# mgtools/DCTdomain

Measured on AMD Instinct MI355X. Metric: DCT fingerprints/sec on L=500 D=1280, higher is better.
Workload: dtype f64

## Files before the change

### dctdomain_amd/csrc/dctfp.hip

```cpp
#include "dctfp.h"

#include <hip/hip_runtime.h>

#include <dlfcn.h>
#include <execinfo.h>
#include <signal.h>
#include <unistd.h>

#include <algorithm>
#include <cmath>
#include <cstdarg>
#include <cstdio>
#include <cstring>
#include <map>
#include <mutex>
#include <new>
#include <string>
#include <unordered_map>
#include <vector>

#include "launch.h"
#include "reccut_kernel.hip.h"

using namespace dctfp;
// ... 2007 lines not shown
                    sp.row_end = row;
                    sp.stripe = stripe++;
                }
            }
        }
    }
    const int64_t used_stripes = s_fill;
    rc = tables.upload(up_bytes, stream, all_bytes);
    if (rc) return rc;
    const TopkJob* djobs = (const TopkJob*)tables.dev();
    const bool long_beside = n_long > 0 && used_stripes > 0 && n_short > 0;
    hipStream_t long_stream = stream;
    if (long_beside) {
        rc = ctx->ensure_cut_streams();
        if (rc == DCTFP_OK) rc = fork.fork(ctx->cut_fork);
        if (rc == DCTFP_OK) rc = fork.branch(ctx->cut[0], &long_stream);
        if (rc) return rc;
    }
    if (n_short > 0) {
        if (ctx->opt_topk_kernel != 1) {
            if (ctx->opt_topk_kernel == 0) {
                constexpr int kSmallK = 1400;
                bool any_small = false, any_large = false;
                for (int32_t q = 0; q < n_short; ++q) (h[q].k <= kSmallK ? any_small : any_large) = true;
                if (any_small)
                    hipLaunchKernelGGL((contact_topk1_kernel<8>), dim3((unsigned)n_short), dim3(512), 0, stream, djobs, out_i, out_j, out_v, out_n, 0, kSmallK);
                if (any_large)
                    hipLaunchKernelGGL((contact_topk1_kernel<16>), dim3((unsigned)n_short), dim3(1024), 0, stream, djobs, out_i, out_j, out_v, out_n,
                                       kSmallK + 1, 0x7fffffff);
            }
            hipLaunchKernelGGL(contact_topk2_kernel, dim3((unsigned)n_short), dim3(1024), 0, stream, djobs, out_i, out_j, out_v, out_n,
                               ctx->opt_topk_kernel == 0 ? 1 : 0);
            hipLaunchKernelGGL(contact_topk_kernel, dim3((unsigned)n_short), dim3(1024), 0, stream, djobs, out_i, out_j, out_v, out_n, 1);
        } else {
            hipLaunchKernelGGL(contact_topk_kernel, dim3((unsigned)n_short), dim3(1024), 0, stream, djobs, out_i, out_j, out_v, out_n, 0);
        }
        HIP_TRY(hipGetLastError());
    }
    if (n_long > 0 && used_stripes > 0) {
        stream = long_stream;
        const TopkJob* dlong = djobs + n_short;
        const TopkStripe* dstripes = (const TopkStripe*)(tables.dev() + off_stripe);
        const int32_t* dfirst = (const int32_t*)(tables.dev() + off_first);
        TopkState* dstate = (TopkState*)(tables.dev() + off_state);
        int32_t* dties = (int32_t*)(tables.dev() + off_ties);
        for (int shift = 24; shift >= 0; shift -= 8) {
            hipLaunchKernelGGL(topk_hist_kernel, dim3((unsigned)used_stripes), dim3(1024), 0, stream, dlong, dstripes, dstate, shift);
            hipLaunchKernelGGL(topk_pick_kernel, dim3((unsigned)n_long), dim3(64), 0, stream, dlong, dstate, shift, out_n);
        }
        hipLaunchKernelGGL(topk_collect_kernel, dim3((unsigned)used_stripes), dim3(1024), 0, stream, dlong, dstripes, dstate, dties, out_i,
                           out_j, out_v);
        hipLaunchKernelGGL(topk_ties_kernel, dim3((unsigned)used_stripes), dim3(64), 0, stream, dlong, dstripes, dstate, dties, dfirst,
                           out_i, out_j, out_v);
        HIP_TRY(hipGetLastError());
    }
    rc = fork.join();
    return rc ? rc : tables.release();
} DCTFP_GUARD("dctfp_contact_topk")

int dctfp_contact_sort(dctfp_ctx* ctx, const void* const* maps, const int64_t* ld, const int32_t* n_res, int32_t n_prot,
                       double t, int32_t* out_i, int32_t* out_j, float* out_v, const int64_t* out_offs, uint8_t* sorted,
                       void* stream_v) try {
    if (!ctx || !maps || !ld || !n_res || !out_i || !out_j || !out_v || !out_offs || !sorted)
        return fail(DCTFP_ERR_INVALID, "dctfp_contact_sort: NULL argument");
    std::lock_guard<std::mutex> lock(ctx->mu);
    if (n_prot < 0) return fail(DCTFP_ERR_INVALID, "dctfp_contact_sort: negative count");
    if (n_prot == 0) return DCTFP_OK;
    hipStream_t stream = (hipStream_t)stream_v;
    HIP_TRY(hipSetDevice(ctx->device));
    static const int kNet[4] = {2048, 4096, 8192, 16384};
    std::vector<int32_t> group[4];
    for (int32_t p = 0; p < n_prot; ++p) {
        const int64_t k = dctfp_contact_count(n_res[p], t);
        sorted[p] = 1;
        if (k <= 1) continue;
        if (n_res[p] > 65536 || k > kNet[3]) {
            sorted[p] = 0;
            continue;
        }
        if (!maps[p] || ld[p] < n_res[p]) return fail(DCTFP_ERR_INVALID, "dctfp_contact_sort: protein %d: bad map", p);
        int g = 0;
        while (k > kNet[g]) ++g;
        group[g].push_back(p);
    }
    const size_t n_jobs = group[0].size() + group[1].size() + group[2].size() + group[3].size();
    if (n_jobs == 0) return DCTFP_OK;
    TableLease tables(ctx->ring, stream);
    int rc = tables.stage(n_jobs * sizeof(TopkJob));
    if (rc) return rc;
    TopkJob* h = (TopkJob*)tables.host();
    size_t q = 0;
    for (int g = 0; g < 4; ++g)
        for (int32_t p : group[g]) {
            h[q].map = (const float*)maps[p];
            h[q].ld = ld[p];
            h[q].n_res = n_res[p];
            h[q].k = (int32_t)dctfp_contact_count(n_res[p], t);
            h[q].out_off = out_offs[p];
            h[q].orig = p;
            h[q].reserved = 0;
            ++q;
        }
    rc = tables.upload(n_jobs * sizeof(TopkJob), stream);
    if (rc) return rc;
    const TopkJob* d = (const TopkJob*)tables.dev();
    size_t first = 0;
    for (int g = 0; g < 4; ++g) {
        const unsigned n = (unsigned)group[g].size();
        if (n == 0) continue;
        if (g == 0) hipLaunchKernelGGL((contact_sort_kernel<2048>), dim3(n), dim3(1024), 0, stream, d + first, out_i, out_j, out_v);
        else if (g == 1) hipLaunchKernelGGL((contact_sort_kernel<4096>), dim3(n), dim3(1024), 0, stream, d + first, out_i, out_j, out_v);
        else if (g == 2) hipLaunchKernelGGL((contact_sort_kernel<8192>), dim3(n), dim3(1024), 0, stream, d + first, out_i, out_j, out_v);
        else hipLaunchKernelGGL((contact_sort_kernel<16384>), dim3(n), dim3(1024), 0, stream, d + first, out_i, out_j, out_v);
        HIP_TRY(hipGetLastError());
        first += n;
    }
    return tables.release();
} DCTFP_GUARD("dctfp_contact_sort")

int64_t dctfp_reccut_room(int32_t n_res) {
    const int64_t doms = n_res > 0 ? n_res / kCutMinSize + 1 : 1;
    return 2 + doms + 2 * (2 * doms + 1);
}

int dctfp_reccut(dctfp_ctx* ctx, const int32_t* n_res, int32_t n_prot, const int32_t* ci, const int32_t* cj, const float* cv,
                 const int64_t* offs, double cut1, double cut2, int32_t* out, const int64_t* out_offs, void* stream_v) try {
    if (!ctx || !n_res || !offs || !out || !out_offs) return fail(DCTFP_ERR_INVALID, "dctfp_reccut: NULL argument");
    std::lock_guard<std::mutex> lock(ctx->mu);
    if (n_prot < 0) return fail(DCTFP_ERR_INVALID, "dctfp_reccut: negative count");
    if (n_prot == 0) return DCTFP_OK;
    hipStream_t stream = (hipStream_t)stream_v;
    HIP_TRY(hipSetDevice(ctx->device));
    std::vector<int32_t> order((size_t)n_prot);
    int32_t count[kCutClasses] = {};
    std::vector<uint8_t> cls((size_t)n_prot);
    size_t adj_total = 0;
    for (int32_t p = 0; p < n_prot; ++p) {
        const int64_t nc = offs[p + 1] - offs[p];
        if (n_res[p] < 0 || nc < 0 || nc > 0x7fffffff || (nc > 0 && (!ci || !cj || !cv)))
            return fail(DCTFP_ERR_INVALID, "dctfp_reccut: protein %d: bad sizes", p);
        if (out_offs[p + 1] - out_offs[p] < 4) return fail(DCTFP_ERR_INVALID, "dctfp_reccut: protein %d: output room below 4", p);
        cls[(size_t)p] = (uint8_t)reccut_class_of(n_res[p], nc);
        ++count[cls[(size_t)p]];
        adj_total += 2 * (size_t)nc + 6 * (size_t)std::max(n_res[p], 0);
    }
    int32_t first[kCutClasses];
    {
        int32_t at[kCutClasses], run = 0;
        for (int c = 0; c < kCutClasses; ++c) {
            first[c] = at[c] = run;
            run += count[c];
        }
        for (int32_t p = 0; p < n_prot; ++p) order[(size_t)at[cls[(size_t)p]]++] = p;
    }
    const size_t stack_ints = (size_t)kCutStack * kCutNodeInts;
    const size_t ws_bytes = align_up(adj_total * sizeof(uint32_t), 16) + (size_t)n_prot * stack_ints * sizeof(int32_t);
    Hold cut_ws{ctx->cut_ws, stream};
    int rc = cut_ws.take(ws_bytes, stream);
    if (rc) return rc;
    TableLease tables(ctx->ring, stream);
    Fork fork(stream);
    rc = tables.stage((size_t)n_prot * sizeof(CutJob));
    if (rc) return rc;
    CutJob* h = (CutJob*)tables.host();
    uint32_t* adj = (uint32_t*)cut_ws.p();
    int32_t* stacks = (int32_t*)((char*)cut_ws.p() + align_up(adj_total * sizeof(uint32_t), 16));
    size_t adj_at = 0;
    for (int32_t q = 0; q < n_prot; ++q) {
        const int32_t p = order[(size_t)q];
        const int64_t nc = offs[p + 1] - offs[p];
        CutJob& j = h[q];
        j.ci = ci ? ci + offs[p] : nullptr;
        j.cj = cj ? cj + offs[p] : nullptr;
        j.cv = cv ? cv + offs[p] : nullptr;
        j.adj = adj + adj_at;
        adj_at += 2 * (size_t)nc + 6 * (size_t)std::max(n_res[p], 0);
        j.stack = stacks + (size_t)q * stack_ints;
        j.out = out + out_offs[p];
        j.timing = nullptr;
#ifdef DCTFP_CUT_TIMING
        j.timing = ctx->degenerate + 1;
#endif
        j.n_contacts = (int32_t)nc;
        j.n_res = n_res[p];
        j.out_cap = (int32_t)std::min<int64_t>(out_offs[p + 1] - out_offs[p], 0x7fffffff);
        j.reserved = 0;
    }
    rc = tables.upload((size_t)n_prot * sizeof(CutJob), stream);
    if (rc) return rc;
    const CutJob* d = (const CutJob*)tables.dev();
    int n_used = 0;
    for (int c = 0; c < kCutClasses; ++c) n_used += count[c] > 0 ? 1 : 0;
    const bool beside = n_used > 1;
    if (beside) {
        rc = ctx->ensure_cut_streams();
        if (rc == DCTFP_OK) rc = fork.fork(ctx->cut_fork);
        if (rc) return rc;
    }
    for (int c = 0; c < kCutClasses; ++c) {
        if (count[c] == 0) continue;
        hipStream_t s = stream;
        if (beside && c > 0) rc = fork.branch(ctx->cut[c - 1], &s);
        if (rc) return rc;
        for (int32_t done = 0; done < count[c]; done += 65535 * 16) {
            const unsigned n = (unsigned)std::min<int32_t>(count[c] - done, 65535 * 16);
            LaunchError le;
            rc = launcher_rc(launch_reccut(c, d + first[c] + done, n, cut1, cut2, s, &le), le);
            if (rc) return rc;
            HIP_TRY(hipGetLastError());
        }
        rc = fork.join();
        if (rc) return rc;
    }
    rc = cut_ws.give_back();
    return rc ? rc : tables.release();
} DCTFP_GUARD("dctfp_reccut")

}

namespace {
struct StitchOnce {
    const float* prev;
    int64_t ld_prev;
    int32_t n_skip;
};
int stitch_impl(dctfp_ctx* ctx, const dctfp_stitch_job* jobs, int64_t n_jobs, int32_t n_cols, int32_t square, void* stream_v,
                const StitchOnce* once = nullptr) {
    if (n_jobs < 0 || (!square && n_cols < 1)) return fail(DCTFP_ERR_INVALID, "dctfp_stitch: bad count");
    if (n_jobs == 0) return DCTFP_OK;
    if (n_jobs > 65535 * 64) return fail(DCTFP_ERR_LIMIT, "dctfp_stitch: too many windows in one call");
    hipStream_t stream = (hipStream_t)stream_v;
    HIP_TRY(hipSetDevice(ctx->device));
    int32_t max_level = 0;
    bool vec4 = !square && n_cols % 4 == 0;
    for (int64_t i = 0; i < n_jobs; ++i) {
        const dctfp_stitch_job& j = jobs[i];
        if (!aligned16(j.src) || !aligned16(j.dst) || (j.ld_src % 4) || (j.ld_dst % 4)) vec4 = false;
        if (once && once[i].prev && (!aligned16(once[i].prev) || (once[i].ld_prev % 4))) vec4 = false;
        if (!j.src || !j.dst || j.n_rows < 1 || j.n_avg < 0 || j.n_avg > j.n_rows || j.level < 0 ||
            j.ld_src < (square ? j.n_rows : n_cols) || j.ld_dst < (square ? j.n_rows : n_cols))
            return fail(DCTFP_ERR_INVALID, "dctfp_stitch: window %lld is malformed", (long long)i);
        if (j.level == 0 && j.n_avg != 0) return fail(DCTFP_ERR_INVALID, "dctfp_stitch: window %lld: level 0 cannot average", (long long)i);
        max_level = std::max(max_level, j.level);
    }
    if (once) max_level = 0;
    TableLease tables(ctx->ring, stream);
    int rc = tables.stage((size_t)n_jobs * sizeof(StitchJob));
    if (rc) return rc;
    StitchJob* h = (StitchJob*)tables.host();
    std::vector<int64_t> start((size_t)max_level + 2, 0);
    for (int64_t i = 0; i < n_jobs; ++i) start[(size_t)(once ? 0 : jobs[i].level) + 1] += 1;
    for (int32_t l = 0; l <= max_level; ++l) start[(size_t)l + 1] += start[(size_t)l];
    std::vector<int64_t> fill(start.begin(), start.end() - 1);
    std::vector<int32_t> max_rows((size_t)max_level + 1, 0);
    for (int64_t i = 0; i < n_jobs; ++i) {
        const dctfp_stitch_job& j = jobs[i];
        const int32_t level = once ? 0 : j.level;
        StitchJob& o = h[fill[(size_t)level]++];
        o.src = (const float*)j.src;
        o.dst = (float*)j.dst;
        o.n_rows = j.n_rows;
        o.n_avg = j.n_avg;
        o.ld_src = j.ld_src;
        o.ld_dst = j.ld_dst;
        o.prev = once ? once[i].prev : nullptr;
        o.ld_prev = once ? once[i].ld_prev : 0;
        o.n_skip = once ? once[i].n_skip : 0;
        o.reserved = 0;
        max_rows[(size_t)level] = std::max(max_rows[(size_t)level], j.n_rows);
    }
    rc = tables.upload((size_t)n_jobs * sizeof(StitchJob), stream);
    if (rc) return rc;
    const StitchJob* d = (const StitchJob*)tables.dev();
    for (int32_t l = 0; l <= max_level; ++l) {
        int64_t cnt = start[(size_t)l + 1] - start[(size_t)l];
        int64_t done = 0;
        while (done < cnt) {
            const unsigned ny = (unsigned)std::min<int64_t>(cnt - done, 65535);
            dim3 grid((unsigned)((max_rows[(size_t)l] + 15) / 16), ny);
            if (square) hipLaunchKernelGGL(stitch_contacts_kernel, grid, dim3(256), 0, stream, d + start[(size_t)l] + done);
            else if (vec4) hipLaunchKernelGGL((stitch_rows_kernel<true>), grid, dim3(256), 0, stream, d + start[(size_t)l] + done, n_cols);
            else hipLaunchKernelGGL((stitch_rows_kernel<false>), grid, dim3(256), 0, stream, d + start[(size_t)l] + done, n_cols);
            HIP_TRY(hipGetLastError());
            done += ny;
        }
    }
    return tables.release();
}

}

extern "C" {

int dctfp_stitch(dctfp_ctx* ctx, const dctfp_stitch_job* jobs, int64_t n_jobs, int32_t n_cols, int32_t square,
                 void* stream_v) try {
    if (!ctx || (!jobs && n_jobs > 0)) return fail(DCTFP_ERR_INVALID, "dctfp_stitch: NULL argument");
    std::lock_guard<std::mutex> lock(ctx->mu);
    return stitch_impl(ctx, jobs, n_jobs, n_cols, square, stream_v);
} DCTFP_GUARD("dctfp_stitch")

int dctfp_stitch_sizes(const int32_t* win_rows, const int64_t* seq_win, int64_t n_seq, int32_t step, int32_t square,
                       int64_t* out_rows) try {
    if (!win_rows || !seq_win || !out_rows || n_seq < 0 || step < 0) return fail(DCTFP_ERR_INVALID, "dctfp_stitch_sizes: bad argument");
    for (int64_t s = 0; s < n_seq; ++s) {
        const int64_t n = seq_win[s + 1] - seq_win[s];
        out_rows[s] = stitch_geometry(win_rows + seq_win[s], n, step, square != 0, [](int64_t, int64_t, int32_t) {});
// ... 558 lines not shown
```

### dctdomain_amd/csrc/reccut_kernel.hip.h

```cpp
#pragma once

#include <hip/hip_runtime.h>
#include <stdint.h>

namespace dctfp {

constexpr int kCutMinTerminal = 10;
constexpr int kCutMinSize = 22;
constexpr int kCutMaxSeg = 24;
constexpr int kCutStack = 24;
constexpr int kCutNodeInts = 4 + 2 * kCutMaxSeg + kCutMaxSeg;

struct CutJob {
    const int32_t* ci;
    const int32_t* cj;
    const float* cv;
    uint32_t* adj;
    int32_t* stack;
    int32_t* out;
    unsigned long long* timing;
    int32_t n_contacts;
    int32_t n_res;
    int32_t out_cap;
    int32_t reserved;
};

__host__ __device__ inline int contact_weight_exact(float p) {
    const double n6 = rint((double)p * 1.0e6);
    const double v = n6 / 1.0e6;
#ifdef __HIP_DEVICE_COMPILE__
    return (int)__dadd_rn(__dmul_rn(v, 100.0), 0.5);
#else
    volatile double prod = v * 100.0;
    return (int)(prod + 0.5);
#endif
}

template <int kCutThreads>
__device__ inline void block_scan_inclusive(int32_t* __restrict__ v, int n, int32_t* __restrict__ wave_tot) {
    const int tid = threadIdx.x, lane = tid & 63, wave = tid >> 6;
    constexpr int NW = kCutThreads / 64;
    int base = 0;
    for (int c0 = 0; c0 < n; c0 += kCutThreads) {
        const int p = c0 + tid;
        int x = p < n ? v[p] : 0;
#pragma unroll
        for (int off = 1; off < 64; off <<= 1) {
            const int up = __shfl_up(x, off);
            x += lane >= off ? up : 0;
        }
        if (lane == 63) wave_tot[wave] = x;
        __syncthreads();
        int before = base;
        for (int w = 0; w < wave; ++w) before += wave_tot[w];
        int total = 0;
        for (int w = 0; w < NW; ++w) total += wave_tot[w];
        if (p < n) v[p] = x + before;
        base += total;
        __syncthreads();
    }
}

__device__ inline bool cut_better(double a, int i, int j, double b, int bi, int bj) {
    return a < b || (a == b && (i < bi || (i == bi && j < bj)));
}

template <int CAP, int ECAP, int kCutThreads, int RB, int KMAX>
__global__ __launch_bounds__(kCutThreads, 4 ) void reccut_kernel(const CutJob* __restrict__ jobs, double cut1, double cut2) {
    extern __shared__ int32_t lds[];
    int32_t* __restrict__ idx = lds;
    int32_t* __restrict__ tmp = idx + CAP;
    int32_t* __restrict__ pos = tmp + CAP;
    int32_t* __restrict__ off = pos + CAP;
    int32_t* __restrict__ foff = off + CAP + 1;
    int32_t* __restrict__ A = foff + CAP + 1;
    int32_t* __restrict__ B = A + CAP + 1;
    uint32_t* __restrict__ fwd = reinterpret_cast<uint32_t*>(B + CAP + 2);
    int32_t* __restrict__ node = reinterpret_cast<int32_t*>(fwd + ECAP);
    int32_t* __restrict__ kid = node + kCutNodeInts;
    int32_t* __restrict__ wtot = kid + 2 * kCutNodeInts;
    int32_t* __restrict__ U = wtot + 32;
    uint8_t* __restrict__ M = reinterpret_cast<uint8_t*>(U + RB * (CAP / 64 + 1));
    int32_t* __restrict__ INITX = reinterpret_cast<int32_t*>(M + RB * CAP);
    auto INIT = [&](int b) -> int32_t* { return b == 0 ? pos : INITX + (b - 1) * CAP; };
    int32_t* __restrict__ WT = INITX + (KMAX > 2 ? KMAX - 2 : 0) * CAP;
    constexpr int RBS = RB / KMAX;
    constexpr int SLOTS = (KMAX * (CAP / 64) / 2 + (CAP / 64) / 2 + 2 * KMAX + kCutThreads / 64 - 1) / (kCutThreads / 64);
    static_assert(RB % KMAX == 0 && RBS % 4 == 0 && RBS * KMAX * 1 <= kCutThreads, "tile rows: RBS rows of each of KMAX bands");
    int32_t* __restrict__ misc = wtot + 16;
    __shared__ double red_ave[kCutThreads / 64];
    __shared__ int red_i[kCutThreads / 64], red_j[kCutThreads / 64];

    const CutJob job = jobs[blockIdx.x];
    const int tid = threadIdx.x, lane = tid & 63, wave = tid >> 6;
    const int L = job.n_res;
    int32_t* __restrict__ out = job.out;
#ifdef DCTFP_CUT_TIMING
    unsigned long long tl_prev = __builtin_amdgcn_s_memrealtime(), tl_acc[11] = {0, 0, 0, 0, 0, 0, 0, 0, 0, 0, 0};
#define CUT_T(k)                                                          \
    do {                                                                  \
        const unsigned long long now_ = __builtin_amdgcn_s_memrealtime(); \
        tl_acc[k] += now_ - tl_prev;                                      \
        tl_prev = now_;                                                   \
    } while (0)
#define CUT_T_OUT()                                                                     \
    do {                                                                                \
        if (tid == 0 && job.timing)                                                     \
            for (int q_ = 0; q_ < 11; ++q_) atomicAdd(job.timing + q_, tl_acc[q_]);      \
    } while (0)
#else
#define CUT_T(k)
#define CUT_T_OUT()
#endif
    if (L < kCutMinSize) {
        if (tid == 0 && job.out_cap >= 4) {
            out[0] = 1;
            out[1] = 1;
            out[2] = 0;
            out[3] = L - 1;
        } else if (tid == 0 && job.out_cap >= 1) {
            out[0] = -1;
        }
        return;
    }
    if (L > CAP || (int64_t)job.n_contacts + 3ll * L > ECAP || job.out_cap < 4) {
        if (tid == 0 && job.out_cap >= 1) out[0] = -1;
        return;
    }
    if (tid < 16) misc[tid] = 0;
    for (int q = tid; q < RB * CAP / 4; q += kCutThreads) reinterpret_cast<uint32_t*>(M)[q] = 0;
    for (int q = tid; q < RB * (CAP / 64 + 1); q += kCutThreads) U[q] = 0;
    __syncthreads();

    for (int r = tid; r < L; r += kCutThreads) {
        int d = 0;
        for (int s = 1; s <= 3; ++s) d += (r - s >= 0 ? 1 : 0) + (r + s < L ? 1 : 0);
        tmp[r] = d;
        idx[r] = r;
        pos[r] = -1;
    }
    __syncthreads();
    for (int c = tid; c < job.n_contacts; c += kCutThreads) {
        const int i = job.ci[c], j = job.cj[c];
        const float p = job.cv[c];
        if (i < 0 || j < 0 || i >= L || j >= L || !(fabsf(p) < 1.0e6f)) {
            misc[4] = 1;
            continue;
        }
        const int d = i > j ? i - j : j - i;
        if (d == 0 || d <= 3) continue;
        if (contact_weight_exact(p) == 0) continue;
        atomicAdd(&tmp[i], 1);
        atomicAdd(&tmp[j], 1);
    }
    __syncthreads();
    for (int r = tid; r < L; r += kCutThreads) A[r] = tmp[r];
    __syncthreads();
    block_scan_inclusive<kCutThreads>(A, L, wtot);
    for (int r = tid; r < L; r += kCutThreads) {
        const int begin = A[r] - tmp[r];
        off[r] = begin;
        if (r == L - 1) off[L] = A[r];
        int at = begin;
        for (int s = 1; s <= 3; ++s) {
            if (r - s >= 0) job.adj[at++] = (uint32_t)(r - s) | (100u << 16);
            if (r + s < L) job.adj[at++] = (uint32_t)(r + s) | (100u << 16);
        }
        B[r] = at;
    }
    __syncthreads();
    if (misc[4] == 0)
        for (int c = tid; c < job.n_contacts; c += kCutThreads) {
            const int i = job.ci[c], j = job.cj[c];
            const int d = i > j ? i - j : j - i;
            if (d <= 3) continue;
            const int w = contact_weight_exact(job.cv[c]);
            if (w == 0) continue;
            if (w < 0 || w > 255) {
                misc[4] = 1;
                continue;
            }
            job.adj[atomicAdd(&B[i], 1)] = (uint32_t)j | ((uint32_t)w << 16);
            job.adj[atomicAdd(&B[j], 1)] = (uint32_t)i | ((uint32_t)w << 16);
        }
    __threadfence_block();
    __syncthreads();
    if (misc[4] != 0) {
        if (tid == 0) out[0] = -1;
        return;
    }
    CUT_T(0);
    if (tid == 0) {
        node[0] = 0;
        node[1] = L;
        node[2] = 1;
        node[3] = 0;
        node[4] = 0;
        node[5] = L - 1;
        misc[9] = 1;
        misc[10] = 0;
        misc[11] = 0;
    }
    __syncthreads();

    for (;;) {
        const int first = node[0], V = node[1];
        int32_t* __restrict__ ix = idx + first;
        for (int p = tid; p < V; p += kCutThreads) pos[ix[p]] = p;
        __syncthreads();
        for (int p = tid; p < V; p += kCutThreads) {
            const int r = ix[p];
            int pre = 0, post = 0, fd = 0;
            for (int e = off[r]; e < off[r + 1]; ++e) {
                const uint32_t a = job.adj[e];
                const int q = pos[a & 0xffffu];
                if (q >= 0) {
                    const int w = (int)(a >> 16);
                    if (q < p) pre += w;
                    else {
                        post += w;
                        ++fd;
                    }
                }
            }
            A[p] = pre;
            B[p] = post;
            foff[p] = fd;
            tmp[p] = fd;
        }
        __syncthreads();
        block_scan_inclusive<kCutThreads>(foff, V, wtot);
        const int n_fwd = foff[V - 1];
        if (n_fwd > ECAP) {
            if (tid == 0) out[0] = -1;
            return;
        }
        for (int p = tid; p < V; p += kCutThreads) {
            const int r = ix[p];
            int at = foff[p] - tmp[p];
            for (int e = off[r]; e < off[r + 1]; ++e) {
                const uint32_t a = job.adj[e];
                const int q = pos[a & 0xffffu];
                if (q > p) fwd[at++] = (uint32_t)q | (a & 0xffff0000u);
            }
        }
        __syncthreads();
        for (int p = tid; p < V; p += kCutThreads) foff[p] = foff[p] - tmp[p];
        CUT_T(1);
        const int post0 = B[0];
        __syncthreads();
        if (tid == 0) {
            A[0] = 0;
            B[0] = 0;
        }
        __syncthreads();
        block_scan_inclusive<kCutThreads>(A, V, wtot);
        block_scan_inclusive<kCutThreads>(B, V, wtot);
        const int sum = B[V - 1] + post0;
        double b1 = 2.0;
        int b1i = 0x7fffffff;
        for (int i = tid; i < V; i += kCutThreads) {
            const int n1 = A[i], spost = B[i];
            const int n2 = sum - spost;
            if (i >= 1 && i < V - 2) {
                const int cutv = post0 + spost - n1;
                const double ave = ((double)cutv) * sum / n1 / n2;
                if (ave < 2.0 && cut_better(ave, i, 0, b1, b1i, 0)) {
                    b1 = ave;
                    b1i = i;
                }
            }
        }
        __syncthreads();
        for (int i = tid; i < V; i += kCutThreads) B[i] = sum - B[i];
        if (tid == 0) B[V] = 0;
        __syncthreads();
        int tj_keep[(CAP + kCutThreads - 1) / kCutThreads], ci_keep[(CAP + kCutThreads - 1) / kCutThreads];
#pragma unroll
        for (int m = 0; m < (CAP + kCutThreads - 1) / kCutThreads; ++m) {
            const int i = m * kCutThreads + tid;
            tj_keep[m] = i < V ? A[i] - B[i + 1] : 0;
            ci_keep[m] = i >= 1 && i < V ? B[i] - A[i - 1] : 0;
        }
        __syncthreads();
#pragma unroll
        for (int m = 0; m < (CAP + kCutThreads - 1) / kCutThreads; ++m) {
            const int i = m * kCutThreads + tid;
            if (i < V) {
                A[i] = tj_keep[m];
                B[i] = ci_keep[m];
            }
        }
        {
#pragma unroll
            for (int o = 32; o >= 1; o >>= 1) {
                const double oa = __shfl_xor(b1, o);
                const int oi = __shfl_xor(b1i, o);
                if (cut_better(oa, oi, 0, b1, b1i, 0)) {
                    b1 = oa;
                    b1i = oi;
                }
            }
            if (lane == 0) {
                red_ave[wave] = b1;
                red_i[wave] = b1i;
            }
        }
        __syncthreads();
        double best1 = 2.0;
        int cuts = 0;
        {
            int bi = 0x7fffffff;
            for (int w = 0; w < kCutThreads / 64; ++w)
                if (cut_better(red_ave[w], red_i[w], 0, best1, bi, 0)) {
                    best1 = red_ave[w];
                    bi = red_i[w];
                }
            if (bi != 0x7fffffff) cuts = bi + 1;
        }
        __syncthreads();
        CUT_T(2);
        double b2 = 2.0;
        int b2i = 0x7fffffff, b2j = 0x7fffffff;
        const bool small = sum > 0 && sum < (1 << 23);
        const float sum_f = (float)sum;
        const int j_end = V - kCutMinTerminal;
        constexpr int NG = CAP / 64, NWV = kCutThreads / 64;
        const int hi_top = j_end - 2;
        const int n_scan_rows = hi_top - kCutMinTerminal + 1;
        int K = n_scan_rows / 16;
        K = K < 1 ? 1 : (K > KMAX ? KMAX : K);
        int band_rows = n_scan_rows > 0 ? (n_scan_rows + K - 1) / K : RBS;
        band_rows = (band_rows + RBS - 1) / RBS * RBS;
        const int n_iter = n_scan_rows > 0 ? band_rows / RBS : 0;
        const int NGa = (j_end + 63) >> 6;
        auto band_top = [&](int b) { return hi_top - b * band_rows; };
        auto band_low = [&](int b) { return max(kCutMinTerminal, hi_top - (b + 1) * band_rows + 1); };
        if (KMAX > 1 && K > 1) {
            for (int b = 0; b < K - 1; ++b)
                for (int q = tid; q < V; q += kCutThreads) INIT(b)[q] = 0;
            __syncthreads();
            for (int a = tid; a <= hi_top; a += kCutThreads) {
                if (a < kCutMinTerminal + 1) continue;
                const int bb = (hi_top - a) / band_rows + 1;
                if (bb >= K) continue;
                const int e1 = foff[a] + tmp[a];
                for (int e = foff[a]; e < e1; ++e) {
                    const uint32_t ent = fwd[e];
                    atomicAdd(&INIT(bb - 1)[(int)(ent & 0xffffu)], (int)(ent >> 16));
                }
            }
            __syncthreads();
            {
                constexpr int PER = (CAP + kCutThreads - 1) / kCutThreads;
                int carry[KMAX > 1 ? KMAX - 1 : 1];
#pragma unroll
                for (int b = 0; b < KMAX - 1; ++b) carry[b] = 0;
#pragma unroll
                for (int m = 0; m < PER; ++m) {
                    const int q = m * kCutThreads + tid;
                    int x[KMAX > 1 ? KMAX - 1 : 1];
                    int run = 0;
#pragma unroll
                    for (int b = 0; b < KMAX - 1; ++b) {
                        run += (b < K - 1 && q < V) ? INIT(b)[q] : 0;
                        x[b] = run;
                    }
#pragma unroll
                    for (int off2 = 1; off2 < 64; off2 <<= 1) {
#pragma unroll
                        for (int b = 0; b < KMAX - 1; ++b) {
                            const int up = __shfl_up(x[b], off2);
                            x[b] += lane >= off2 ? up : 0;
                        }
                    }
                    if (lane == 63) {
#pragma unroll
                        for (int b = 0; b < KMAX - 1; ++b) WT[b * NWV + wave] = x[b];
                    }
                    __syncthreads();
#pragma unroll
                    for (int b = 0; b < KMAX - 1; ++b) {
                        int before = carry[b], total = 0;
                        for (int w = 0; w < NWV; ++w) {
                            const int t_w = WT[b * NWV + w];
                            before += w < wave ? t_w : 0;
                            total += t_w;
                        }
                        if (b < K - 1 && q < V) INIT(b)[q] = x[b] + before;
                        carry[b] += total;
                    }
                    __syncthreads();
                }
            }
        }
        int n_tasks = 0;
        int cum[KMAX + 1];
#pragma unroll
        for (int b = 0; b < KMAX; ++b) {
            cum[b] = n_tasks;
            if (b < K && n_scan_rows > 0 && band_top(b) >= kCutMinTerminal) {
                const int g_lo = (band_low(b) + 1) >> 6;
                n_tasks += max(0, NGa - g_lo);
            }
        }
        cum[KMAX] = n_tasks;
        int task_b[SLOTS], task_g[SLOTS], below[SLOTS];
#pragma unroll
        for (int sl = 0; sl < SLOTS; ++sl) {
            const int tau = wave + sl * NWV;
            int b = -1, g = 0;
            if (tau < n_tasks) {
#pragma unroll
                for (int bb = 0; bb < KMAX; ++bb)
                    if (tau >= cum[bb] && tau < cum[bb + 1]) {
                        b = bb;
                        g = ((band_low(bb) + 1) >> 6) + tau - cum[bb];
                    }
            }
            task_b[sl] = b;
            task_g[sl] = g;
            const int j = g * 64 + lane;
            below[sl] = (b >= 1 && j < j_end) ? INIT(b - 1)[j] : 0;
        }
        if (n_tasks > SLOTS * NWV) {
            if (tid == 0) out[0] = -1;
            return;
        }
        float best_f = 2.0f * 1.0001f;
        for (int it = 0; it < n_iter; ++it) {
            constexpr int FPR = kCutThreads / (KMAX * RBS) >= 8 ? 8 : kCutThreads / (KMAX * RBS);
            const int fill_t = tid / FPR, fill_b = fill_t / RBS;
            int fill_row = -1;
            if (fill_b < K) {
                const int r = band_top(fill_b) - it * RBS - (fill_t % RBS);
                if (r >= band_low(fill_b)) fill_row = r;
            }
            if (fill_row >= 0) {
                const int e1 = foff[fill_row] + tmp[fill_row];
                for (int e = foff[fill_row] + tid % FPR; e < e1; e += FPR) {
                    const uint32_t ent = fwd[e];
                    const int q = (int)(ent & 0xffffu);
                    M[fill_t * CAP + q] = (uint8_t)(ent >> 16);
                    atomicAdd(&U[fill_t * (NG + 1) + (q >> 6)], (int)(ent >> 16));
                }
            }
            __syncthreads();
            CUT_T(3);
#pragma unroll
            for (int sl = 0; sl < SLOTS; ++sl) {
                const int b = task_b[sl], g = task_g[sl];
                if (b < 0) continue;
                const int hi = band_top(b) - it * RBS;
                const int n_rows = min(RBS, hi - band_low(b) + 1);
                const int g0 = g * 64;
                if (n_rows <= 0 || g0 + 63 <= hi - n_rows + 1) continue;
                const int j = g0 + lane;
                const bool col_ok = j < j_end;
                const int tj = col_ok ? A[j] : 0;
                const int tr0 = b * RBS;
                int m_u = 0;
                if (lane < n_rows)
                    for (int k = 0; k < g; ++k) m_u += U[(tr0 + lane) * (NG + 1) + k];
                const int m_c = lane < n_rows ? B[hi - lane] : 0;
                int bl = below[sl];
                static_assert(RBS % 4 == 0, "rows go through four at a time");
                for (int t = 0; t < n_rows; t += 4) {
                    int x[4], ns2[4], cv[4], ns1[4];
                    bool maybe[4];
#pragma unroll
                    for (int k = 0; k < 4; ++k) x[k] = (int)M[(tr0 + t + k) * CAP + j];
#pragma unroll
                    for (int k = 0; k < 4; ++k) {
                        x[k] += __builtin_amdgcn_update_dpp(0, x[k], 0x111, 0xf, 0xf, true);
                        x[k] += __builtin_amdgcn_update_dpp(0, x[k], 0x112, 0xf, 0xf, true);
                        x[k] += __builtin_amdgcn_update_dpp(0, x[k], 0x114, 0xf, 0xf, true);
                        x[k] += __builtin_amdgcn_update_dpp(0, x[k], 0x118, 0xf, 0xf, true);
                        x[k] += __builtin_amdgcn_update_dpp(0, x[k], 0x142, 0xa, 0xf, false);
                        x[k] += __builtin_amdgcn_update_dpp(0, x[k], 0x143, 0xc, 0xf, false);
                    }
                    bool any = false;
#pragma unroll
                    for (int k = 0; k < 4; ++k) {
                        bl += x[k] + __builtin_amdgcn_readlane(m_u, min(t + k, 63));
                        const int i = hi - t - k;
                        ns2[k] = bl;
                        cv[k] = tj + __builtin_amdgcn_readlane(m_c, min(t + k, 63)) - 2 * bl;
                        ns1[k] = sum - cv[k] - bl;
                        maybe[k] = t + k < n_rows && col_ok && j - i >= kCutMinSize - 1 && ns1[k] > 0 && ns2[k] > 0;
                        if (small) maybe[k] = maybe[k] && (float)cv[k] * sum_f <= best_f * (float)ns1[k] * (float)ns2[k];
                        any |= maybe[k];
                    }
                    if (__builtin_amdgcn_ballot_w64(any) != 0) {
                        bool improved = false;
#pragma unroll
                        for (int k = 0; k < 4; ++k)
                            if (maybe[k]) {
                                const double ave = ((double)cv[k]) * sum / ns1[k] / ns2[k];
                                if (ave < 2.0 && cut_better(ave, hi - t - k, j, b2, b2i, b2j)) {
                                    b2 = ave;
                                    b2i = hi - t - k;
                                    b2j = j;
                                    improved = true;
                                }
                            }
                        if (__builtin_amdgcn_ballot_w64(improved) != 0) {
                            double wmin = b2;
#pragma unroll
                            for (int o = 32; o >= 1; o >>= 1) wmin = fmin(wmin, __shfl_xor(wmin, o));
                            best_f = (float)(wmin * 1.0001);
                        }
                    }
                }
                below[sl] = bl;
            }
            CUT_T(8);
            __syncthreads();
            CUT_T(9);
            if (fill_row >= 0) {
                const int e1 = foff[fill_row] + tmp[fill_row];
                for (int e = foff[fill_row] + tid % FPR; e < e1; e += FPR) {
                    const int q = (int)(fwd[e] & 0xffffu);
                    M[fill_t * CAP + q] = 0;
                    U[fill_t * (NG + 1) + (q >> 6)] = 0;
                }
            }
            __syncthreads();
            CUT_T(10);
        }
#pragma unroll
        for (int o = 32; o >= 1; o >>= 1) {
            const double oa = __shfl_xor(b2, o);
            const int oi = __shfl_xor(b2i, o), oj = __shfl_xor(b2j, o);
            if (cut_better(oa, oi, oj, b2, b2i, b2j)) {
                b2 = oa;
                b2i = oi;
                b2j = oj;
            }
        }
        if (lane == 0) {
            red_ave[wave] = b2;
            red_i[wave] = b2i;
            red_j[wave] = b2j;
        }
        __syncthreads();
        CUT_T(3);
        if (tid == 0) {
            double best2 = 2.0;
            int cuts1 = 0x7fffffff, cuts2 = 0x7fffffff;
            for (int w = 0; w < kCutThreads / 64; ++w)
                if (cut_better(red_ave[w], red_i[w], red_j[w], best2, cuts1, cuts2)) {
                    best2 = red_ave[w];
                    cuts1 = red_i[w];
                    cuts2 = red_j[w];
                }
            if (cuts1 == 0x7fffffff) cuts1 = cuts2 = 0;
            const int n_seg = node[2], n_site = node[3];
            const int32_t* __restrict__ segs = node + 4;
            const int32_t* __restrict__ sites = node + 4 + 2 * kCutMaxSeg;
            int action = 0;
            int32_t* __restrict__ k1 = kid;
            int32_t* __restrict__ k2 = kid + kCutNodeInts;
            int n1s = 0, n1c = 0, n2s = 0, n2c = 0;
            bool bad = false;
            auto seg_ok = [&](int c) { return c >= 0 && c < n_seg; };
            auto push_seg = [&](int32_t* __restrict__ k, int& n, int a, int b) {
                if (n >= kCutMaxSeg) {
                    bad = true;
                    return;
                }
                k[4 + 2 * n] = a;
                k[4 + 2 * n + 1] = b;
                ++n;
            };
            auto push_site = [&](int32_t* __restrict__ k, int& n, int v) {
                if (n >= kCutMaxSeg) {
                    bad = true;
                    return;
                }
                k[4 + 2 * kCutMaxSeg + n] = v;
                ++n;
            };
            if (best1 - cut1 <= best2 - cut2) {
                if (!(best1 > cut1 || cuts < kCutMinSize || V - cuts < kCutMinSize)) {
                    action = 1;
                    int c = 0;
                    while (c < n_site && sites[c] < cuts) {
                        if (!seg_ok(c)) bad = true;
                        else push_seg(k1, n1s, segs[2 * c], segs[2 * c + 1]);
                        push_site(k1, n1c, sites[c]);
                        ++c;
                        if (bad) break;
                    }
                    if (!bad && !seg_ok(c)) bad = true;
                    if (!bad) {
                        const int len1 = c == 0 ? cuts : cuts - sites[c - 1];
                        const int mf = segs[2 * c], ms = segs[2 * c + 1];
                        push_seg(k1, n1s, mf, mf + len1 - 1);
                        const int len2 = (n_site == 0 || c == n_site) ? V - cuts : sites[c] - cuts;
                        if (len2 > 0) {
                            push_seg(k2, n2s, ms - len2 + 1, ms);
                            if (c < n_site) push_site(k2, n2c, len2);
                        }
                        for (++c; c < n_seg; ++c) {
                            push_seg(k2, n2s, segs[2 * c], segs[2 * c + 1]);
                            if (c < n_site && len1 > 0) push_site(k2, n2c, len1);
                        }
                    }
                    k1[1] = cuts;
                    k2[1] = V - cuts;
                }
            } else {
                const int length = cuts2 - cuts1;
                if (!(best2 > cut2 || length < kCutMinSize || V - length < kCutMinSize)) {
                    action = 2;
                    const int ns = n_site;
                    const int tail = V - cuts2;
                    int c1 = -1, c2 = 0;
                    for (int i = ns - 1; i >= 0; --i) {
                        if (sites[i] < cuts2) c2 = i + 1;
                        if (sites[i] <= cuts1) {
                            c1 = i;
                            break;
                        }
                    }
                    auto cs_at = [&](int i) {
                        if (i == -1 && ns > 0) return 0;
                        if (i < 0 || i >= ns) {
                            bad = true;
                            return 0;
                        }
                        return sites[i];
                    };
                    const int len2 = c2 == 0 ? cuts2 : cuts2 - cs_at(c2 - 1);
                    if (!seg_ok(c2)) bad = true;
                    if (!bad) {
                        push_seg(k1, n1s, segs[2 * c2] + len2, segs[2 * c2 + 1]);
                        for (int i = c2 + 1; i <= ns && !bad; ++i) {
                            if (!seg_ok(i)) bad = true;
                            else push_seg(k1, n1s, segs[2 * i], segs[2 * i + 1]);
                        }
                        for (int i = c2; i < ns; ++i) push_site(k1, n1c, sites[i] - cuts2);
                        push_site(k1, n1c, tail);
                        for (int i = 0; i <= c1 && !bad; ++i) {
                            if (!seg_ok(i)) bad = true;
                            else push_seg(k1, n1s, segs[2 * i], segs[2 * i + 1]);
                            if (sites[i] != cuts1) push_site(k1, n1c, sites[i] + tail);
                        }
                    }
                    if (!bad) {
                        const int len1 = c1 >= 0 ? cuts1 - sites[c1] : cuts1;
                        ++c1;
                        if (len1 > 0) {
                            if (!seg_ok(c1)) bad = true;
                            else push_seg(k1, n1s, segs[2 * c1], segs[2 * c1] + len1 - 1);
                        }
                        if (!bad && c2 > c1) {
                            const int lhs = cs_at(c1 - 1) + len1, rhs = cs_at(c1);
                            if (!bad && lhs < rhs) {
                                if (!seg_ok(c1)) bad = true;
                                else push_seg(k2, n2s, segs[2 * c1] + len1, segs[2 * c1 + 1]);
                            }
                        }
                        for (int i = c1 + 1; i < c2 && !bad; ++i) {
                            if (!seg_ok(i)) bad = true;
                            else push_seg(k2, n2s, segs[2 * i], segs[2 * i + 1]);
                        }
                        if (!bad) {
                            if (c2 > c1 && len2 > 0) {
                                if (!seg_ok(c2)) bad = true;
                                else push_seg(k2, n2s, segs[2 * c2], segs[2 * c2] + len2 - 1);
                            } else if (c1 == c2) {
                                if (!seg_ok(c2)) bad = true;
                                else push_seg(k2, n2s, segs[2 * c2] + len1, segs[2 * c2] + len2 - 1);
                            }
                        }
                        for (int i = c1; i < c2 && !bad; ++i) {
                            const int v = cs_at(i) - cuts1;
                            if (!bad && v > 0) push_site(k2, n2c, v);
                        }
// ... 94 lines not shown
```

Before: 1.373 million.

## Pack row prefix scans, drop barriers, sort cut jobs by size

After: 1.373 million (median of 6 runs). No clear change (-0.0%).

```diff
diff --git a/dctdomain_amd/csrc/dctfp.hip b/dctdomain_amd/csrc/dctfp.hip
--- a/dctdomain_amd/csrc/dctfp.hip
+++ b/dctdomain_amd/csrc/dctfp.hip
@@ -2183,6 +2183,10 @@
             run += count[c];
         }
         for (int32_t p = 0; p < n_prot; ++p) order[(size_t)at[cls[(size_t)p]]++] = p;
+        for (int c = 0; c < kCutClasses; ++c)
+            std::stable_sort(order.begin() + first[c], order.begin() + first[c] + count[c], [&](int32_t a, int32_t b) {
+                return (int64_t)n_res[a] * n_res[a] > (int64_t)n_res[b] * n_res[b];
+            });
     }
     const size_t stack_ints = (size_t)kCutStack * kCutNodeInts;
     const size_t ws_bytes = align_up(adj_total * sizeof(uint32_t), 16) + (size_t)n_prot * stack_ints * sizeof(int32_t);
diff --git a/dctdomain_amd/csrc/reccut_kernel.hip.h b/dctdomain_amd/csrc/reccut_kernel.hip.h
--- a/dctdomain_amd/csrc/reccut_kernel.hip.h
+++ b/dctdomain_amd/csrc/reccut_kernel.hip.h
@@ -88,8 +88,8 @@
     constexpr int SLOTS = (KMAX * (CAP / 64) / 2 + (CAP / 64) / 2 + 2 * KMAX + kCutThreads / 64 - 1) / (kCutThreads / 64);
     static_assert(RB % KMAX == 0 && RBS % 4 == 0 && RBS * KMAX * 1 <= kCutThreads, "tile rows: RBS rows of each of KMAX bands");
     int32_t* __restrict__ misc = wtot + 16;
-    __shared__ double red_ave[kCutThreads / 64];
-    __shared__ int red_i[kCutThreads / 64], red_j[kCutThreads / 64];
+    __shared__ double red_ave[kCutThreads / 64], red1_ave[kCutThreads / 64];
+    __shared__ int red_i[kCutThreads / 64], red_j[kCutThreads / 64], red1_i[kCutThreads / 64];
 
     const CutJob job = jobs[blockIdx.x];
     const int tid = threadIdx.x, lane = tid & 63, wave = tid >> 6;
@@ -302,8 +302,8 @@
                 }
             }
             if (lane == 0) {
-                red_ave[wave] = b1;
-                red_i[wave] = b1i;
+                red1_ave[wave] = b1;
+                red1_i[wave] = b1i;
             }
         }
         __syncthreads();
@@ -312,13 +312,12 @@
         {
             int bi = 0x7fffffff;
             for (int w = 0; w < kCutThreads / 64; ++w)
-                if (cut_better(red_ave[w], red_i[w], 0, best1, bi, 0)) {
-                    best1 = red_ave[w];
-                    bi = red_i[w];
+                if (cut_better(red1_ave[w], red1_i[w], 0, best1, bi, 0)) {
+                    best1 = red1_ave[w];
+                    bi = red1_i[w];
                 }
             if (bi != 0x7fffffff) cuts = bi + 1;
         }
-        __syncthreads();
         CUT_T(2);
         double b2 = 2.0;
         int b2i = 0x7fffffff, b2j = 0x7fffffff;
@@ -430,6 +429,7 @@
         float best_f = 2.0f * 1.0001f;
         for (int it = 0; it < n_iter; ++it) {
             constexpr int FPR = kCutThreads / (KMAX * RBS) >= 8 ? 8 : kCutThreads / (KMAX * RBS);
+            static_assert(64 % FPR == 0, "a tile row's fill threads lie in one wave");
             const int fill_t = tid / FPR, fill_b = fill_t / RBS;
             int fill_row = -1;
             if (fill_b < K) {
@@ -468,16 +468,23 @@
                 for (int t = 0; t < n_rows; t += 4) {
                     int x[4], ns2[4], cv[4], ns1[4];
                     bool maybe[4];
-#pragma unroll
-                    for (int k = 0; k < 4; ++k) x[k] = (int)M[(tr0 + t + k) * CAP + j];
-#pragma unroll
-                    for (int k = 0; k < 4; ++k) {
-                        x[k] += __builtin_amdgcn_update_dpp(0, x[k], 0x111, 0xf, 0xf, true);
-                        x[k] += __builtin_amdgcn_update_dpp(0, x[k], 0x112, 0xf, 0xf, true);
-                        x[k] += __builtin_amdgcn_update_dpp(0, x[k], 0x114, 0xf, 0xf, true);
-                        x[k] += __builtin_amdgcn_update_dpp(0, x[k], 0x118, 0xf, 0xf, true);
-                        x[k] += __builtin_amdgcn_update_dpp(0, x[k], 0x142, 0xa, 0xf, false);
-                        x[k] += __builtin_amdgcn_update_dpp(0, x[k], 0x143, 0xc, 0xf, false);
+                    uint32_t xp[2];
+#pragma unroll
+                    for (int h = 0; h < 2; ++h)
+                        xp[h] = (uint32_t)M[(tr0 + t + 2 * h) * CAP + j] | ((uint32_t)M[(tr0 + t + 2 * h + 1) * CAP + j] << 16);
+#pragma unroll
+                    for (int h = 0; h < 2; ++h) {
+                        xp[h] += __builtin_amdgcn_update_dpp(0u, xp[h], 0x111, 0xf, 0xf, true);
+                        xp[h] += __builtin_amdgcn_update_dpp(0u, xp[h], 0x112, 0xf, 0xf, true);
+                        xp[h] += __builtin_amdgcn_update_dpp(0u, xp[h], 0x114, 0xf, 0xf, true);
+                        xp[h] += __builtin_amdgcn_update_dpp(0u, xp[h], 0x118, 0xf, 0xf, true);
+                        xp[h] += __builtin_amdgcn_update_dpp(0u, xp[h], 0x142, 0xa, 0xf, false);
+                        xp[h] += __builtin_amdgcn_update_dpp(0u, xp[h], 0x143, 0xc, 0xf, false);
+                    }
+#pragma unroll
+                    for (int h = 0; h < 2; ++h) {
+                        x[2 * h] = (int)(xp[h] & 0xffffu);
+                        x[2 * h + 1] = (int)(xp[h] >> 16);
                     }
                     bool any = false;
 #pragma unroll
@@ -525,7 +532,6 @@
                     U[fill_t * (NG + 1) + (q >> 6)] = 0;
                 }
             }
-            __syncthreads();
             CUT_T(10);
         }
 #pragma unroll
```
